# cbg-ethz/metMHN

Measured on AMD Instinct MI355X. Metric: full-cohort log-lik+grad evals/sec at n=20 events; kronvec HBM GB/s, higher is better.
Workload: dtype f64

## Files before the change

### include/metmhn_amd.h

```cpp
#ifndef METMHN_AMD_H
#define METMHN_AMD_H

#include <stddef.h>
#include <stdint.h>

#ifdef __cplusplus
extern "C" {
#endif

typedef struct mmhn_engine* mmhn_handle;

enum { MMHN_F64 = 0, MMHN_F32 = 1 };

int mmhn_create(int device_id, int n_mut, int dtype, mmhn_handle* out);
void mmhn_destroy(mmhn_handle h);
const char* mmhn_last_error(void);
int mmhn_set_workspace_limit(mmhn_handle h, size_t bytes);

int mmhn_set_cohort(mmhn_handle h, const int8_t* dat, int64_t n_pat, int n_cols);
int mmhn_score(mmhn_handle h, const double* log_theta, const double* log_d_p, const double* log_d_m,
               double perc_met, double* score);
int mmhn_score_and_grad(mmhn_handle h, const double* log_theta, const double* log_d_p,
                        const double* log_d_m, double perc_met, double* score, double* d_theta,
                        double* d_dp, double* d_dm);
// ... 59 lines not shown

enum { MMHN_ORD_OK = 0, MMHN_ORD_OVERFLOW = 1, MMHN_ORD_INVALID = 2, MMHN_ORD_TOO_LARGE = 3 };
enum { MMHN_ORD_BAD_STATUS = 1,
       MMHN_ORD_UNREACHABLE = 2,
       MMHN_ORD_NO_SEEDING = 3,
       MMHN_ORD_MT_PT_PART = 4,
       MMHN_ORD_MT_NO_SEEDING = 5,
       MMHN_ORD_ABSENT_MET = 6,
       MMHN_ORD_PRESENT_MET = 7 };
enum { MMHN_ORD_DEFAULT_FRONT_CAP = 64 };
int mmhn_likeliest_orders(mmhn_handle h, const double* log_theta, const double* obs1, const double* obs2,
                          const int8_t* dat, int64_t n_pat, int n_cols, int front_cap, int8_t* orders, double* prob,
                          int32_t* status);

enum { MMHN_K_OTHER_SOLVE = 0,
       MMHN_K_PSOLVE_FWD = 1,
       MMHN_K_PSOLVE_ADJ = 2,
       MMHN_K_PCLASS = 3,
       MMHN_K_CSOLVE_FWD = 4,
       MMHN_K_CSOLVE_ADJ = 5,
       MMHN_K_COUNT = 6 };
typedef struct {
  double ms;
  int64_t launches;
  double alg_bytes;
} mmhn_kernel_counter;
typedef struct {
  mmhn_kernel_counter kernel[MMHN_K_COUNT];
  double eval_ms;
  int64_t evals;
  int32_t comm_ranks;
  int32_t comm_rank;
} mmhn_counters;
#define MMHN_ABI_VERSION 7
int mmhn_abi_version(void);
int mmhn_bench_kronvec(mmhn_handle h, const double* log_theta, const int8_t* state, int64_t batch,
                       int iters, int transpose, int jacobi, double* ms_per_launch, int64_t* tiles);
int mmhn_bench_stream(mmhn_handle h, size_t bytes, int iters, int kind, double* gbps);
int mmhn_get_counters(mmhn_handle h, mmhn_counters* out);
int mmhn_reset_counters(mmhn_handle h);
int mmhn_debug_lane_moves(mmhn_handle h, int transposed, int* out);

#ifdef __cplusplus
}
#endif
#endif
```

### metmhn_amd/_lib.py

```python
from __future__ import annotations

import ctypes as C
import os
import subprocess

_HERE = os.path.dirname(os.path.abspath(__file__))
_ROOT = os.path.dirname(_HERE)
import glob
_SRC = [os.path.join(_HERE, "csrc", "engine.hip")] + sorted(glob.glob(os.path.join(_HERE, "csrc", "*.h")))
_HDR = os.path.join(_ROOT, "include", "metmhn_amd.h")
LIB_PATH = os.environ.get("MMHN_LIB", os.path.join(_HERE, "libmetmhn_amd.so"))

f64p = C.POINTER(C.c_double)
i8p = C.POINTER(C.c_int8)
i64p = C.POINTER(C.c_int64)
i32p = C.POINTER(C.c_int32)


KERNEL_CLASSES = ("other_solve", "psolve_fwd", "psolve_adj", "pclass", "csolve_fwd", "csolve_adj")


class KernelCounter(C.Structure):
    _fields_ = [("ms", C.c_double), ("launches", C.c_int64), ("alg_bytes", C.c_double)]

# ... 14 lines not shown
    "mmhn_cohort_sums_end": [C.c_void_p, f64p],
    "mmhn_cohort_wsums_begin": [C.c_void_p, f64p, f64p, f64p, C.c_int, C.c_double],
    "mmhn_cohort_wsums_end": [C.c_void_p, f64p],
    "mmhn_set_reduce_flag": [C.c_void_p, C.c_double],
    "mmhn_get_reduce_flag": [C.c_void_p, f64p],
    "mmhn_patient_grads": [C.c_void_p, f64p, f64p, f64p, f64p, f64p, f64p, f64p],
    "mmhn_kronvec": [C.c_void_p, f64p, i8p, f64p, f64p, C.c_int, C.c_int],
    "mmhn_kronvec_batched": [C.c_void_p, f64p, i8p, C.c_int64, f64p, f64p, C.c_int, C.c_int],
    "mmhn_jacobi_step_batched": [C.c_void_p, f64p, f64p, f64p, i8p, C.c_int64, f64p, f64p, f64p, C.c_int],
    "mmhn_kron_diag": [C.c_void_p, f64p, i8p, f64p],
    "mmhn_diag_scal": [C.c_void_p, f64p, i8p, f64p, f64p, C.c_int],
    "mmhn_obs_states": [C.c_void_p, i8p, C.c_int, i64p, i64p],
    "mmhn_resolvent": [C.c_void_p, f64p, f64p, f64p, i8p, f64p, f64p, C.c_int],
    "mmhn_x_partial_Q_y": [C.c_void_p, f64p, i8p, f64p, f64p, f64p],
    "mmhn_x_partial_D_y": [C.c_void_p, f64p, f64p, i8p, f64p, f64p, f64p, f64p],
    "mmhn_partial_diag_scal": [C.c_void_p, f64p, i8p, f64p, C.c_int, C.c_int, f64p],
    "mmhn_v_kronvec": [C.c_void_p, f64p, i8p, f64p, f64p, C.c_int, C.c_int],
    "mmhn_v_resolvent": [C.c_void_p, f64p, i8p, f64p, f64p, f64p, C.c_int],
    "mmhn_v_x_partial_Q_y": [C.c_void_p, f64p, i8p, f64p, f64p, f64p, f64p],
    "mmhn_v_kron_diag": [C.c_void_p, f64p, i8p, f64p, f64p],
    "mmhn_v_scal_d_pt": [C.c_void_p, f64p, f64p, i8p, f64p, f64p, f64p],
    "mmhn_v_d_scal_d_pt": [C.c_void_p, f64p, f64p, i8p, f64p, C.c_int, f64p, f64p],
    "mmhn_v_x_partial_D_y": [C.c_void_p, f64p, f64p, i8p, f64p, f64p, f64p, f64p],
    "mmhn_comm_unique_id": [C.c_void_p],
    "mmhn_comm_init": [C.c_void_p, C.c_void_p, C.c_int, C.c_int],
    "mmhn_comm_destroy": [C.c_void_p],
    "mmhn_bench_stream": [C.c_void_p, C.c_size_t, C.c_int, C.c_int, f64p],
    "mmhn_bench_kronvec": [C.c_void_p, f64p, i8p, C.c_int64, C.c_int, C.c_int, C.c_int, f64p, i64p],
    "mmhn_simulate": [C.c_void_p, f64p, f64p, f64p, C.c_int64, C.c_uint64, i8p, i8p],
    "mmhn_simulate_summary": [C.c_void_p, f64p, f64p, f64p, C.c_int64, C.c_int64, C.c_uint64, i64p],
    "mmhn_get_counters": [C.c_void_p, C.POINTER(Counters)],
    "mmhn_reset_counters": [C.c_void_p],
    "mmhn_debug_lane_moves": [C.c_void_p, C.c_int, C.POINTER(C.c_int)],
    "mmhn_likeliest_orders": [C.c_void_p, f64p, f64p, f64p, i8p, C.c_int64, C.c_int, C.c_int, i8p, f64p, i32p],
}
OTHER_SYMBOLS = ("mmhn_destroy", "mmhn_last_error", "mmhn_abi_version")
ABI_VERSION = 7


def needs_build() -> bool:
    if not os.path.exists(LIB_PATH):
        return True
    t = os.path.getmtime(LIB_PATH)
    return any(os.path.exists(s) and os.path.getmtime(s) > t for s in _SRC + [_HDR])


def build(force: bool = False, verbose: bool = False) -> str:
    if not force and not needs_build():
        return LIB_PATH
    hipcc = os.environ.get("HIPCC", "/opt/rocm/bin/hipcc")
    cmd = [hipcc, "-O3", "-std=c++17", "--offload-arch=gfx950", "-shared", "-fPIC", "-Wno-comment",
           "-o", LIB_PATH, _SRC[0]]
    if verbose:
        print(" ".join(cmd))
    res = subprocess.run(cmd, capture_output=True, text=True)
    if res.returncode != 0:
        raise RuntimeError("hipcc failed:\n" + res.stderr)
    return LIB_PATH


_lib = None


def load():
    global _lib
    if _lib is not None:
        return _lib
    if not os.path.exists(LIB_PATH):
        raise RuntimeError(
            f"{LIB_PATH} is missing: run `python -c 'import __graft_entry__ as g; g.build()'` "
# ... 30 lines not shown
```

### metmhn_amd/csrc/engine.hip

```cpp
#include <hip/hip_runtime.h>
#include <rccl/rccl.h>
#include <dlfcn.h>

#include <algorithm>
#include <chrono>
#include <cmath>
#include <cstdio>
#include <cstdlib>
#include <cstring>
#include <string>
#include <vector>

#include "../../include/metmhn_amd.h"
#include "kernels.h"
#include "tsolve.h"
#include "small.h"
#include "wsolve.h"
#include "wclass.h"
#include "sampler.h"

namespace mmhn {

static thread_local std::string g_err;

// ... 52 lines not shown

struct Staged {
  std::vector<int> pats, paired, probs;
  DevArr<int> d_pats, d_paired, d_probs;
  std::vector<int2> map, lmap;
  std::vector<int> lof;
  DevArr<int2> d_map, d_lmap;
  DevArr<int2> d_grc;
  CList cl[2];
  int maxk = 0;
  bool kind2 = false;
  bool empty() const { return pats.empty(); }
};

struct Batch {
  std::vector<PatRec> pats;
  std::vector<Desc> dJ, dS;
  std::vector<int2> mapJ, mapS;
  long long vecJ = 0, vecS = 0, asize = 0, tabJ = 0, tabS = 0;
  long long aclr = 0;
  int id = 0;
  int maxkJ = 0, maxkS = 0;
  int maxkcJ = 0;
  bool has_kind2 = false;
  std::vector<int2> lmapJ, lmapS;
  std::vector<int> lofJ, lofS;
  std::vector<int2> mapX;
  DevArr<int2> d_mapX;
  DevArr<int2> d_grc[4];
  DevArr<int2> d_grcJ;
  std::vector<int> sp_list[3][SP_NCLASS];
  DevArr<int> d_sp_list[3][SP_NCLASS];
  bool has_small = false;
  int mk1p = 9;
  Staged stg[2];
  std::vector<int> paired;
  DevArr<int> d_paired;
  std::vector<uint8_t> route;
  std::vector<int> olist;
  DevArr<int> d_olist;
  bool wpath = false;
  bool wdirect = false;
  std::vector<WDesc> wd;
  DevArr<WDesc> d_wd;
  int wnx = -1;
  std::vector<WChain> wchains;
  DevArr<WChain> d_wchains;
  long long offT = 0;
  CList clJ[2];
  std::vector<int2> lmapT;
  std::vector<int> lofT;
  DevArr<int2> d_lmapT;
  int maxkT = 0, maxkP = 0;
  int max_dl = 0;
  std::vector<int> ptoff;
  std::vector<uint32_t> ptiles;
  DevArr<int> d_ptoff;
  DevArr<uint32_t> d_ptiles;
  double seeded_bytes_P = 0;
  std::vector<int4> pcl;
  DevArr<int4> d_pcl;
  DevArr<PatRec> d_pats;
  DevArr<Desc> d_dJ, d_dS;
  DevArr<int2> d_mapJ, d_mapS, d_lmapJ, d_lmapS;
};

// ... 252 lines not shown
template <typename T>
struct Engine : EngineBase {
  int n = 0, N = 0;
  size_t ws_limit = 0;
  DevArr<Params<T>> d_par;
  Params<T>* h_par = nullptr;
  double* h_abi = nullptr;
  void* h_par_dev = nullptr;
  double* h_abi_dev = nullptr;
  bool zero_copy = true;
  bool time_kernels = true;
  std::vector<int8_t> dat;
  long long n_pat = 0;
  int n_cols = 0;
  std::vector<Batch> batches;
  double n_em = 0;
  DevArr<T> pi, lidgJ, qJ, rhsJ, rhsS, pS, lidgS, qS, seedS, GS, dots, bmJ, bmS, tabJ, tabS;
  DevArr<T> zarena;
  struct View { T* p = nullptr; } GJ, DJ, Abuf;
  static long long zarena_elems(long long nJ, long long asize, int N) { return up4(3 * nJ * N * N) + up4(3 * nJ * N) + up4(asize); }
  static long long zclear_elems(const Batch& b, int N) { return zarena_elems((long long)b.dJ.size(), b.aclr, N); }
  static long long up4(long long v) { return (v + 3) / 4 * 4; }
  int pi_owner = -1, qJ_owner = -1;
  DevArr<double> lp, out, sums, abi_sums, redbuf;
  DevArr<JLink<T>> links;
  ncclComm_t comm = nullptr;
  int comm_rank = 0, comm_size = 1;
  DevArr<uint16_t> d_perm;
  DevArr<int> d_lvl;
  bool use_jacobi = false;
  bool poison = false;
  hipStream_t side[3] = {};
  hipEvent_t ev_fork[3] = {}, ev_join[3] = {};
  bool small_path = true;
  int prep_split_max = 2048;
  int psolve_min = 384;
  int wsolve_min = 128;
  bool force_timing = false;
  bool coop_fault = false;
  int pcl_per = 16;
  int coop_wgs = 0;
  bool coop = true;
  DevArr<CoopCtl> coop_ctl;
  DevArr<unsigned> coop_flags[2];
  unsigned coop_epoch = 0;
  int coop_slot = 0;
  int cur_lane = 0;
  unsigned* h_abort = nullptr;
  unsigned* h_abort_dev = nullptr;
  int wsolve_wgs = 0;
  int wsolve_mode = 1;
  DevArr<T> piM, qM;
  int n_cu = 256;
  mmhn_counters cnt{};
  std::vector<std::pair<hipEvent_t, hipEvent_t>> ev_pool;
  size_t ev_used = 0;
  std::vector<double> ev_bytes;
  std::vector<int> ev_slot;

  Engine(int dev, int n_mut) : n(n_mut), N(n_mut + 1) {
    device = dev;
    cnt.comm_rank = -1;
    REQUIRE(n_mut >= 1 && n_mut < MAXN, "n_mut must be in [1, 31]");
    DevGuard guard(device);
    HIPCHECK(hipStreamCreateWithFlags(&stream, hipStreamNonBlocking));
    d_par.alloc(NPSET);
// ... 1 lines not shown
    HIPCHECK(hipHostGetDevicePointer(&h_par_dev, h_par, 0));
    static_assert(sizeof(Params<T>) % sizeof(uint4) == 0, "parameter block: whole 16-byte words");
    sums.alloc(2 * stride());
    size_t free_b = 0, total_b = 0;
    HIPCHECK(hipMemGetInfo(&free_b, &total_b));
    ws_limit = (size_t)(0.7 * (double)free_b);
    {
      std::vector<uint16_t> perm((size_t)(TB + 1) << TB, 0);
      std::vector<int> lvl((size_t)(TB + 1) * (TB + 2), 0);
      for (int t = 0; t <= TB; ++t) {
        int pos = 0;
        for (int l = 0; l <= t; ++l) {
          lvl[(size_t)t * (TB + 2) + l] = pos;
          for (uint32_t x = 0; x < (1u << t); ++x)
            if (popc(x) == l) perm[((size_t)t << TB) + pos++] = (uint16_t)x;
        }
        lvl[(size_t)t * (TB + 2) + t + 1] = pos;
      }
      d_perm.alloc(perm.size());
      d_lvl.alloc(lvl.size());
      HIPCHECK(hipMemcpy(d_perm.p, perm.data(), perm.size() * sizeof(uint16_t), hipMemcpyHostToDevice));
      HIPCHECK(hipMemcpy(d_lvl.p, lvl.data(), lvl.size() * sizeof(int), hipMemcpyHostToDevice));
      const char* sv = std::getenv("MMHN_SOLVER");
      use_jacobi = sv && std::string(sv) == "jacobi";
      if (const char* pm = std::getenv("MMHN_PSOLVE_MIN")) { psolve_min = std::atoi(pm); wsolve_min = psolve_min; }
      if (const char* pm = std::getenv("MMHN_WSOLVE_MIN")) wsolve_min = std::atoi(pm);
      if (const char* pm = std::getenv("MMHN_COOP")) coop = std::atoi(pm) != 0;
      if (const char* pm = std::getenv("MMHN_TIME_KERNELS")) force_timing = std::atoi(pm) != 0;
      if (const char* pm = std::getenv("MMHN_COOP_WGS")) coop_wgs = std::atoi(pm);
      if (const char* pm = std::getenv("MMHN_PCL_PER")) pcl_per = std::max(1, std::atoi(pm));
      if (const char* pm = std::getenv("MMHN_COOP_FAULT")) coop_fault = std::atoi(pm) != 0;
      if (const char* po = std::getenv("MMHN_POISON")) poison = std::atoi(po) != 0;
      if (const char* sp = std::getenv("MMHN_SMALL")) small_path = std::atoi(sp) != 0;
      if (const char* sp = std::getenv("MMHN_ZEROCOPY")) zero_copy = std::atoi(sp) != 0;
      if (const char* sp = std::getenv("MMHN_PREP_SPLIT")) prep_split_max = std::atoi(sp);
      if (const char* ms = std::getenv("MMHN_WSOLVE")) wsolve_mode = std::atoi(ms);
      if (const char* ms = std::getenv("MMHN_WSOLVE_WGS")) wsolve_wgs = std::atoi(ms);
      if (const char* sc = std::getenv("MMHN_SIM_CHUNK")) sim_chunk = std::max(1ll, std::atoll(sc));
      hipDeviceProp_t prop;
      HIPCHECK(hipGetDeviceProperties(&prop, device));
      n_cu = std::max(1, prop.multiProcessorCount);
    }
    HIPCHECK(hipFuncSetAttribute(reinterpret_cast<const void*>(&k_wsolve<T, false>), hipFuncAttributeMaxDynamicSharedMemorySize, (int)wsolve_lds<T>()));
    HIPCHECK(hipFuncSetAttribute(reinterpret_cast<const void*>(&k_wsolve<T, true>), hipFuncAttributeMaxDynamicSharedMemorySize, (int)wsolve_lds<T>()));
    HIPCHECK(hipFuncSetAttribute(reinterpret_cast<const void*>(&k_wsolve<T, false, WCfg<T>::NXT>), hipFuncAttributeMaxDynamicSharedMemorySize, (int)wsolve_lds<T>()));
    HIPCHECK(hipFuncSetAttribute(reinterpret_cast<const void*>(&k_wsolve<T, true, WCfg<T>::NXT>), hipFuncAttributeMaxDynamicSharedMemorySize, (int)wsolve_lds<T>()));
    HIPCHECK(hipFuncSetAttribute(reinterpret_cast<const void*>(&k_wclass<T>), hipFuncAttributeMaxDynamicSharedMemorySize, (int)wclass_lds<T>()));
    const int lds = 150 * 1024;
    HIPCHECK(hipFuncSetAttribute(reinterpret_cast<const void*>(&k_csolve<T, false, false>), hipFuncAttributeMaxDynamicSharedMemorySize, lds));
    HIPCHECK(hipFuncSetAttribute(reinterpret_cast<const void*>(&k_csolve<T, true, false>), hipFuncAttributeMaxDynamicSharedMemorySize, lds));
    HIPCHECK(hipFuncSetAttribute(reinterpret_cast<const void*>(&k_csolve<T, false, true>), hipFuncAttributeMaxDynamicSharedMemorySize, lds));
    HIPCHECK(hipFuncSetAttribute(reinterpret_cast<const void*>(&k_csolve<T, true, true>), hipFuncAttributeMaxDynamicSharedMemorySize, lds));
    HIPCHECK(hipFuncSetAttribute(reinterpret_cast<const void*>(&k_csolve<T, false, false, 4>), hipFuncAttributeMaxDynamicSharedMemorySize, lds));
    HIPCHECK(hipFuncSetAttribute(reinterpret_cast<const void*>(&k_csolve<T, true, false, 4>), hipFuncAttributeMaxDynamicSharedMemorySize, lds));
    coop_ctl.alloc(1);
    HIPCHECK(hipMemset(coop_ctl.p, 0, sizeof(CoopCtl)));
    HIPCHECK(hipHostMalloc(reinterpret_cast<void**>(&h_abort), 64, hipHostMallocDefault));
    HIPCHECK(hipHostGetDevicePointer(reinterpret_cast<void**>(&h_abort_dev), h_abort, 0));
    *h_abort = 0u;
    HIPCHECK(hipFuncSetAttribute(reinterpret_cast<const void*>(&k_spatient2<T>), hipFuncAttributeMaxDynamicSharedMemorySize, 160 * 1024));
    HIPCHECK(hipFuncSetAttribute(reinterpret_cast<const void*>(&k_spatient<T, 1024, 1>), hipFuncAttributeMaxDynamicSharedMemorySize, 160 * 1024));
    for (int i = 0; i < 3; ++i) {
      HIPCHECK(hipStreamCreateWithFlags(&side[i], hipStreamNonBlocking));
      HIPCHECK(hipEventCreateWithFlags(&ev_fork[i], hipEventDisableTiming));
      HIPCHECK(hipEventCreateWithFlags(&ev_join[i], hipEventDisableTiming));
    }
    HIPCHECK(hipFuncSetAttribute(reinterpret_cast<const void*>(&k_psolve2<T, false, true>), hipFuncAttributeMaxDynamicSharedMemorySize, lds));
    HIPCHECK(hipFuncSetAttribute(reinterpret_cast<const void*>(&k_psolve2<T, true, true>), hipFuncAttributeMaxDynamicSharedMemorySize, lds));
    HIPCHECK(hipFuncSetAttribute(reinterpret_cast<const void*>(&k_psolve2<T, false, false>), hipFuncAttributeMaxDynamicSharedMemorySize, lds));
    HIPCHECK(hipFuncSetAttribute(reinterpret_cast<const void*>(&k_psolve2<T, true, false>), hipFuncAttributeMaxDynamicSharedMemorySize, lds));
    HIPCHECK(hipFuncSetAttribute(reinterpret_cast<const void*>(&k_tsolve<T, false, false>), hipFuncAttributeMaxDynamicSharedMemorySize, lds));
    HIPCHECK(hipFuncSetAttribute(reinterpret_cast<const void*>(&k_tsolve<T, true, false>), hipFuncAttributeMaxDynamicSharedMemorySize, lds));
    HIPCHECK(hipFuncSetAttribute(reinterpret_cast<const void*>(&k_tsolve<T, false, true>), hipFuncAttributeMaxDynamicSharedMemorySize, lds));
    HIPCHECK(hipFuncSetAttribute(reinterpret_cast<const void*>(&k_tsolve<T, true, true>), hipFuncAttributeMaxDynamicSharedMemorySize, lds));
    HIPCHECK(hipFuncSetAttribute(reinterpret_cast<const void*>(&k_kv<T, false, 1, false>), hipFuncAttributeMaxDynamicSharedMemorySize, lds));
    HIPCHECK(hipFuncSetAttribute(reinterpret_cast<const void*>(&k_kv<T, true, 1, false>), hipFuncAttributeMaxDynamicSharedMemorySize, lds));
    HIPCHECK(hipFuncSetAttribute(reinterpret_cast<const void*>(&k_kv<T, false, 1, true>), hipFuncAttributeMaxDynamicSharedMemorySize, lds));
    HIPCHECK(hipFuncSetAttribute(reinterpret_cast<const void*>(&k_kv<T, true, 1, true>), hipFuncAttributeMaxDynamicSharedMemorySize, lds));
    HIPCHECK(hipFuncSetAttribute(reinterpret_cast<const void*>(&k_sweep<T, false>),
                                 hipFuncAttributeMaxDynamicSharedMemorySize, lds));
    HIPCHECK(hipFuncSetAttribute(reinterpret_cast<const void*>(&k_sweep<T, true>),
                                 hipFuncAttributeMaxDynamicSharedMemorySize, lds));
    HIPCHECK(hipFuncSetAttribute(reinterpret_cast<const void*>(&k_diag<T>),
                                 hipFuncAttributeMaxDynamicSharedMemorySize, lds));
    HIPCHECK(hipFuncSetAttribute(reinterpret_cast<const void*>(&k_diag<T, 1024>),
                                 hipFuncAttributeMaxDynamicSharedMemorySize, lds));
    HIPCHECK(hipFuncSetAttribute(reinterpret_cast<const void*>(&k_prep<T, false>), hipFuncAttributeMaxDynamicSharedMemorySize, lds));
    HIPCHECK(hipFuncSetAttribute(reinterpret_cast<const void*>(&k_prep<T, true>), hipFuncAttributeMaxDynamicSharedMemorySize, lds));
    HIPCHECK(hipFuncSetAttribute(reinterpret_cast<const void*>(&k_prep<T, false, 1024>), hipFuncAttributeMaxDynamicSharedMemorySize, lds));
    HIPCHECK(hipFuncSetAttribute(reinterpret_cast<const void*>(&k_grad_rows<T, 1>), hipFuncAttributeMaxDynamicSharedMemorySize, lds));
    HIPCHECK(hipFuncSetAttribute(reinterpret_cast<const void*>(&k_grad_rows<T>),
                                 hipFuncAttributeMaxDynamicSharedMemorySize, lds));
    HIPCHECK(hipFuncSetAttribute(reinterpret_cast<const void*>(&k_pclass<T, false>), hipFuncAttributeMaxDynamicSharedMemorySize, lds));
    HIPCHECK(hipFuncSetAttribute(reinterpret_cast<const void*>(&k_pclass<T, true>), hipFuncAttributeMaxDynamicSharedMemorySize, lds));
// ... 593 lines not shown
      bool class_fits[SP_NCLASS];
      for (int c = 0; c < SP_NCLASS; ++c)
        class_fits[c] = (spatient_lds<T>(N, spatient_class_maxk(c)) + 15) / 16 * 16 * (size_t)(c == 0 ? SP_PPB0 : c == 1 ? 2 : 1) + 64 <= (size_t)160 * 1024;
      const bool all_staged = !small_path || use_jacobi;
      for (size_t pi_ = 0; pi_ < b.pats.size(); ++pi_) {
        const PatRec& pr = b.pats[pi_];
        int ks = -1;
        for (int part = 0; part < 2; ++part) if (pr.s[part] >= 0) ks = std::max(ks, b.dS[pr.s[part]].k);
        if (ks < 0) continue;
        int c = 0;
        while (c < SP_NCLASS - 1 && ks > spatient_class_maxk(c)) ++c;
        if (all_staged || ks > TB || !class_fits[c]) {
          Staged& g = b.stg[all_staged || pr.j >= 0 ? 1 : 0];
          g.pats.push_back((int)pi_);
          if (pr.j >= 0) g.paired.push_back((int)pi_);
          for (int part = 0; part < 2; ++part) if (pr.s[part] >= 0) g.probs.push_back(pr.s[part]);
          if (pr.kind == 2) g.kind2 = true;
          continue;
        }
        const bool side_by_side = pr.j >= 0 && pr.s[0] >= 0 && pr.s[1] >= 0 && c < 2;
        b.sp_list[side_by_side ? 2 : pr.j >= 0 ? 1 : 0][c].push_back((int)pi_);
      }
      b.mk1p = spatient_class_maxk(1);
      if (!b.sp_list[1][2].empty() && b.sp_list[1][2].size() <= 16) {
        int mk = 0;
        for (int pi_ : b.sp_list[1][2])
          for (int part = 0; part < 2; ++part) if (b.pats[pi_].s[part] >= 0) mk = std::max(mk, b.dS[b.pats[pi_].s[part]].k);
        if (mk <= 10 && (spatient_lds<T>(N, mk) + 15) / 16 * 16 * 2 + 64 <= (size_t)160 * 1024) {
          for (int pi_ : b.sp_list[1][2]) b.sp_list[b.pats[pi_].s[0] >= 0 && b.pats[pi_].s[1] >= 0 ? 2 : 1][1].push_back(pi_);
          b.sp_list[1][2].clear();
          b.mk1p = mk;
        }
      }
      {
        auto ksize = [&](int pi_) {
          const PatRec& pr = b.pats[pi_];
          int ks = 0;
          for (int part = 0; part < 2; ++part) if (pr.s[part] >= 0) ks = std::max(ks, 64 * b.dS[pr.s[part]].k + (pr.s[0] >= 0 && pr.s[1] >= 0 ? 32 : 0) + pr.kind);
          return ks;
        };
        for (int w = 0; w < 3; ++w)
          for (int c = 0; c < SP_NCLASS; ++c)
            std::stable_sort(b.sp_list[w][c].begin(), b.sp_list[w][c].end(), [&](int x, int y) { return ksize(x) > ksize(y); });
      }
      b.has_small = false;
      for (int w = 0; w < 3; ++w)
        for (int c = 0; c < SP_NCLASS; ++c) {
          if (!b.sp_list[w][c].empty()) b.has_small = true;
          up(b.d_sp_list[w][c], b.sp_list[w][c]);
        }
      for (int w = 0; w < 2; ++w) {
        Staged& g = b.stg[w];
        std::vector<char> isg(b.dS.size(), 0);
        for (int sp : g.probs) isg[sp] = 1;
        g.map.clear(); g.maxk = 0;
        for (const int2& m : b.mapS) if (isg[m.x]) { g.map.push_back(m); g.maxk = std::max(g.maxk, b.dS[m.x].k); }
        build_levels(g.map, nullptr, false, g.lmap, g.lof);
        g.cl[0].clear(); g.cl[1].clear();
        if (!use_jacobi && g.lof.size() > 2) { build_clist(g.map, b.dS, false, false, g.cl[0]); build_clist(g.map, b.dS, false, true, g.cl[1]); }
        up(g.d_pats, g.pats); up(g.d_paired, g.paired); up(g.d_probs, g.probs);
        up(g.d_map, g.map); up(g.d_lmap, g.lmap);
        std::vector<int2> gc;
        for (const int2& e : grad_chunks(b.dS, GK_S)) if (isg[e.x]) gc.push_back(e);
        up(g.d_grc, gc);
      }
      b.wdirect = b.wpath && wsolve_mode != 2;
// ... 17 lines not shown
          up(b.d_grc[kd], gc);
          if (kd != GK_S) for (int2 e : gc) all.push_back(int2{e.x, e.y | (kd << 24)});
        }
        up(b.d_grcJ, all);
      }
      mvJ = std::max(mvJ, b.vecJ); mvS = std::max(mvS, b.vecS);
      mZ = std::max<size_t>(mZ, (size_t)zarena_elems((long long)b.dJ.size(), b.asize, N));
      mtJ = std::max(mtJ, b.tabJ); mtS = std::max(mtS, b.tabS);
      if (b.wpath && !b.wdirect) mvM = std::max(mvM, b.vecJ);
      mnJ = std::max(mnJ, b.dJ.size()); mnS = std::max(mnS, b.dS.size()); mp = std::max(mp, b.pats.size());
    }
    pi.alloc(mvJ); qJ.alloc(mvJ);
    piM.alloc(mvM); qM.alloc(mvM);
    if (use_jacobi) { lidgJ.alloc(mvJ); rhsJ.alloc(mvJ); }
    links.alloc(std::max<size_t>(mnJ, 1));
    tabJ.alloc(mtJ); tabS.alloc(mtS);
    pi_owner = qJ_owner = -1;
    rhsS.alloc(mvS); pS.alloc(mvS); lidgS.alloc(mvS); qS.alloc(mvS);
    seedS.alloc(mnS);
    GS.alloc(mnS * N * N); zarena.alloc(mZ);
    dots.alloc(2 * mp); bmJ.alloc(mnJ * 64); bmS.alloc(mnS * 64);
    lp.alloc(mp); out.alloc(mp * stride()); redbuf.alloc(((mp + red_per((int)mp) - 1) / red_per((int)mp)) * 2 * (size_t)stride());
  }

  bool small_forked[2] = {false, false}, fork_recorded[2] = {false, false};
  void small_fork(int which) {
    HIPCHECK(hipEventRecord(ev_fork[which], stream));
    fork_recorded[which] = true;
  }
  void small_classes(const Batch& b, int which, bool grad) {
    const int n0 = (int)b.sp_list[which][0].size(), n1 = (int)b.sp_list[which][1].size(), n2 = (int)b.sp_list[which][2].size();
    const int np0 = which ? (int)b.sp_list[2][0].size() : 0, np1 = which ? (int)b.sp_list[2][1].size() : 0;
    const int mk0 = spatient_class_maxk(0), mk1 = which ? b.mk1p : spatient_class_maxk(1), mk2 = spatient_class_maxk(2);
    const bool on_side = which == 0 ? (n0 + n1 + n2 > 0) : n2 > 0;
    hipStream_t sd = side[which];
    if (on_side) {
      if (!fork_recorded[which]) HIPCHECK(hipEventRecord(ev_fork[which], stream));
      HIPCHECK(hipStreamWaitEvent(sd, ev_fork[which], 0));
    }
    fork_recorded[which] = false;
#define SP_TAIL b.d_pats.p, b.d_dS.p, d_par.p, d_perm.p, d_lvl.p, b.d_dJ.p, b.d_wd.p, pi.p, links.p, pS.p, qS.p, GS.p, bmS.p, dots.p, lp.p
    auto big_class = [&]() {
      if (!n2) return;
      const size_t lds = (spatient_lds<T>(N, mk2) + 15) / 16 * 16;
      hipLaunchKernelGGL((k_spatient<T, 1024, 1>), dim3(n2), dim3(1024), lds, sd, b.d_sp_list[which][2].p, n2, SP_TAIL, mk2, N, grad ? 1 : 0);
      HIPCHECK(hipGetLastError());
    };
    big_class();
    if (n0 + n1 + np0 + np1) {
      const size_t s0 = (spatient_lds<T>(N, mk0) + 15) / 16 * 16, s1 = (spatient_lds<T>(N, mk1) + 15) / 16 * 16;
      const size_t lds = std::max(s0 * SP_PPB0, n1 + np1 ? s1 * (np1 ? 2 : 1) : 0) + 64;
      const int nblk = (n0 + SP_PPB0 - 1) / SP_PPB0 + n1 + (np0 + SP_PPB0 / 2 - 1) / (SP_PPB0 / 2) + np1;
      hipLaunchKernelGGL((k_spatient2<T>), dim3(nblk), dim3(256), lds, which == 0 ? sd : stream,
                         b.d_sp_list[which][0].p, n0, mk0, b.d_sp_list[which][1].p, n1, mk1,
                         b.d_sp_list[2][0].p, np0, b.d_sp_list[2][1].p, np1, SP_TAIL, N, grad ? 1 : 0);
      HIPCHECK(hipGetLastError());
    }
#undef SP_TAIL
    if (on_side) HIPCHECK(hipEventRecord(ev_join[which], sd));
    small_forked[which] = on_side;
  }
  void small_join(int which) {
    if (small_forked[which]) HIPCHECK(hipStreamWaitEvent(stream, ev_join[which], 0));
    small_forked[which] = false;
  }

  void evaluate(const double* lt, const double* ldp, const double* ldm, bool grad, double* host_sums,
                double* host_out) {
    REQUIRE(!sums_pending, "an evaluation begun with mmhn_cohort_sums_begin has not been collected");
    auto t0 = std::chrono::steady_clock::now();
    const int st = stride();
    small_forked[0] = small_forked[1] = fork_recorded[0] = fork_recorded[1] = false;
    bool head_done = false;
    if (zero_copy && !batches.empty()) {
      build_params(lt, ldp, ldm, false);
// ... 1243 lines not shown
  GUARD(h);
  unsigned long long v[16];
  HIPCHECK(hipDeviceSynchronize());
  HIPCHECK(hipMemcpyFromSymbol(v, HIP_SYMBOL(g_stamps), sizeof(v)));
  for (int i = 0; i < 16; ++i) out16[i] = (double)v[i];
  if (reset) { std::memset(v, 0, sizeof(v)); HIPCHECK(hipMemcpyToSymbol(HIP_SYMBOL(g_stamps), v, sizeof(v))); }
  API_END
}
#endif
int mmhn_get_counters(mmhn_handle h, mmhn_counters* out) {
  API_BEGIN
  GUARD(h);
  REQUIRE(h && h->impl && out, "null pointer");
  if (h->dtype == MMHN_F64) *out = static_cast<Engine<double>*>(h->impl)->cnt;
  else *out = static_cast<Engine<float>*>(h->impl)->cnt;
  API_END
}
int mmhn_debug_lane_moves(mmhn_handle h, int transposed, int* out) {
  API_BEGIN
  GUARD(h);
  REQUIRE(out, "null pointer");
  DevArr<int> d;
  d.alloc(6 * 64);
  if (transposed) hipLaunchKernelGGL((k_lane_moves<true>), dim3(1), dim3(64), 0, h->impl->stream, d.p);
  else hipLaunchKernelGGL((k_lane_moves<false>), dim3(1), dim3(64), 0, h->impl->stream, d.p);
  HIPCHECK(hipGetLastError());
  HIPCHECK(hipMemcpyAsync(out, d.p, 6 * 64 * sizeof(int), hipMemcpyDeviceToHost, h->impl->stream));
  HIPCHECK(hipStreamSynchronize(h->impl->stream));
  API_END
}

int mmhn_abi_version(void) { return MMHN_ABI_VERSION; }

int mmhn_reset_counters(mmhn_handle h) {
  API_BEGIN
  GUARD(h);
  DISPATCH(h, reset_counters());
  API_END
}

}
```

### metmhn_amd/csrc/small.h

```cpp
#pragma once
#include "kernels.h"

namespace mmhn {

constexpr int SP_NCLASS = 3;
constexpr int SP_PPB0 = 4;
__host__ __device__ inline int spatient_class_maxk(int c) { return c == 0 ? 6 : c == 1 ? 9 : TB; }
__host__ __device__ inline int spatient_lstride(int maxk) { return maxk < 6 ? 1 << maxk : 64; }
__host__ __device__ inline int spatient_rows(int maxk) { return maxk > 6 ? 1 << (maxk - 6) : 1; }

template <typename T>
__host__ __device__ inline size_t spatient_lds(int N, int maxk) {
  return ((size_t)N * (spatient_lstride(maxk) + spatient_rows(maxk) + 16 + 1) + 4 * 64 + 2 * 16 + ((size_t)3 << maxk) + 64) * sizeof(T) +
         (64 + TB + 2) * sizeof(int) + 8 + DESC_PAD + (sizeof(uint16_t) << maxk);
}

template <typename T, int SPB, int PPB, bool PAIR = false>
__device__ __forceinline__ void spatient_body(const int* __restrict__ plist, int npl, const PatRec* __restrict__ pats, const Desc* __restrict__ dS,
                                              const Params<T>* __restrict__ par,
                                              const uint16_t* __restrict__ perm, const int* __restrict__ lvl,
                                              const Desc* __restrict__ dJ, const WDesc* __restrict__ wds, const T* __restrict__ pi, JLink<T>* __restrict__ links,
                                              T* __restrict__ pS, T* __restrict__ qS,
                                              T* __restrict__ GS, T* __restrict__ bmS, T* __restrict__ dots,
                                              double* __restrict__ lp, int maxk, int N, int with_grad, int block) {
  constexpr int SPW = SPB / 64;
  static_assert(PAIR ? (PPB == 2 || (SPB == 64 && PPB % 2 == 0)) : (PPB == 1 || SPB == 64),
                "several patients per workgroup: one wave each; a pair of problems: two slots");
  extern __shared__ __align__(16) unsigned char smem_all[];
  const int pslot = PPB == 1 ? 0 : (int)(threadIdx.x / SPB);
  const size_t slot_bytes = (spatient_lds<T>(N, maxk) + 15) / 16 * 16;
  unsigned char* smem = smem_all + (size_t)pslot * slot_bytes;
  T* xch = reinterpret_cast<T*>(smem_all + (size_t)PPB * slot_bytes);
  const int mypart = pslot & 1;
  auto sync = [&]() {
    if (SPB == 64) { __builtin_amdgcn_fence(__ATOMIC_ACQ_REL, "wavefront"); __builtin_amdgcn_wave_barrier(); }
    else __syncthreads();
  };
  const int RS = spatient_rows(maxk);
  const int LS = spatient_lstride(maxk);
  T* Lc = reinterpret_cast<T*>(smem);
  T* Uc = Lc + N * LS;
  T* LA = Uc + N * RS;
  T* UA = LA + 64;
  T* LB = UA + 64;
  T* UB = LB + 64;
  T* P0 = UB + 64;
  T* Qv = P0 + ((size_t)1 << maxk);
  T* LID = Qv + ((size_t)1 << maxk);
  T* red = LID + ((size_t)1 << maxk);
  T* thl = red + 64;
  T* basel = thl + N * 16;
  T* dpl = basel + N;
  T* dml = dpl + 16;
  int* lev = reinterpret_cast<int*>(dml + 16);
  int* loff = lev + 64;
  Desc& dsh = *reinterpret_cast<Desc*>((reinterpret_cast<uintptr_t>(loff + TB + 2) + 7u) & ~(uintptr_t)7u);
  uint16_t* pml = reinterpret_cast<uint16_t*>(reinterpret_cast<unsigned char*>(&dsh) + DESC_PAD);
  const int pidx = PAIR ? block * (PPB / 2) + (pslot >> 1) : block * PPB + pslot;
  if (pidx >= npl) { if (PAIR && SPB == 64) __syncthreads(); return; }
  const int pat = plist[pidx];
  const PatRec pr = pats[pat];
  const int ps0 = pr.s[0], ps1 = pr.s[1];
  if (pr.kind == 4 || (PAIR ? (ps0 < 0 || ps1 < 0) : (ps0 < 0 && ps1 < 0))) { if (PAIR && SPB == 64) __syncthreads(); return; }
  const int kwalk = (PAIR && SPB > 64) ? max(dS[ps0].k, dS[ps1].k) : -1;
  const int tid = (int)(threadIdx.x % SPB), lane = tid & 63, w = tid >> 6;
  const int n = N - 1;

  auto setup = [&](const Desc& dg) {
    sync();
    {
      const int* sw = reinterpret_cast<const int*>(&dg);
      int* dw = reinterpret_cast<int*>(&dsh);
      for (int i = tid; i < DESC_WORDS; i += SPB) dw[i] = sw[i];
    }
    sync();
    const Desc& d = dsh;
    const int k = d.k;
    const Params<T>& P = par[d.pset];
    const int nl = k < 6 ? k : 6;
    const int R = k > 6 ? 1 << (k - 6) : 1;
    if (tid < k) { lev[tid] = d.ev[tid]; dpl[tid] = P.dp[d.ev[tid]]; dml[tid] = P.dm[d.ev[tid]]; }
    for (int e = tid; e < N * k; e += SPB) { const int i = e / k, b = e % k; thl[i * 16 + b] = P.th[i][d.ev[b]]; }
    for (int i = tid; i < N; i += SPB) basel[i] = P.baseP[i];
    if (SPB > 64) {
      const uint16_t* pm = perm + ((size_t)k << TB);
      for (uint32_t e = tid; e < (1u << k); e += SPB) pml[e] = pm[e];
      if (tid <= k + 1) loff[tid] = lvl[(size_t)k * (TB + 2) + tid];
    }
    sync();
    const int nL = 1 << nl;
    for (int e = tid; e < N * nL; e += SPB) {
      const int i = e >> nl, l = e & (nL - 1);
      T t[6];
#pragma unroll
      for (int bb = 0; bb < 6; ++bb) t[bb] = thl[i * 16 + bb];
      T v = 1;
#pragma unroll
// ... 94 lines not shown
    m.half = 1u << (k - 1);
    m.joff = dj->off;
    m.wl = dj->wl; m.kj = kj;
    m.free_is_row = m.wl >= 0 && (wds[m.wl].majP != 0) == (part == 1);
    return m;
  };
  auto marg_rhs = [&](const Marg& m, uint32_t x) -> T {
    if (x < m.half) return T(0);
    if (m.wl >= 0) return m.c * pi[m.joff + wpos_marg<T>(wds[m.wl], m.kj, m.free_is_row, x - m.half)];
    return m.c * pi[m.joff + (pdep32(x - m.half, m.free_) | m.fixed)];
  };
  Marg mg0{}, mg1{};

  STAMP_DECL;
  STAMP_START;
  T full_score = 0;
  for (int part = 0; part < 2; ++part) {
    const int sp = part == 0 ? ps0 : ps1;
    if (sp < 0 || (PAIR && part != mypart)) continue;
    setup(dS[sp]);
    STAMP(0);
    const Desc& d = dsh;
    const bool own = pr.kind <= 2;
    Marg mg{};
    if (!own) {
      mg = marg_of(part, d.k);
      if (part == 0) mg0 = mg; else mg1 = mg;
      if (tid == 0) { links[pr.j].soff[part] = d.off; links[pr.j].sk[part] = d.k; links[pr.j].cst[part] = mg.c; }
    }
    const bool stash = !PAIR && part == 1 && ps0 >= 0;
    T* yv = stash ? Qv : P0;
    solve(d, yv, false, [&](uint32_t x) { return own ? (x == 0 ? e0_scale<T>() : T(0)) : marg_rhs(mg, x); });
    full_score += yv[(1u << d.k) - 1u];
    if (stash) for (uint32_t x = tid; x < (1u << d.k); x += SPB) pS[d.off + x] = yv[x];
    STAMP(1);
  }
  if (pr.kind == 3 && !PAIR && tid == 0) {
    if (ps0 < 0) { links[pr.j].soff[0] = -1; links[pr.j].sk[0] = 0; links[pr.j].cst[0] = 0; }
    if (ps1 < 0) { links[pr.j].soff[1] = -1; links[pr.j].sk[1] = 0; links[pr.j].cst[1] = 0; }
  }
  if (PAIR) {
    if (tid == 0) xch[pslot] = full_score;
    __syncthreads();
    full_score = xch[pslot & ~1] + xch[pslot | 1];
  }
  const T seed = T(1) / full_score;
  if (tid == 0 && !(PAIR && mypart == 1)) {
    double l = log((double)full_score) - log((double)e0_scale<T>());
    if (pr.kind == 2) {
      const Desc& d = dsh;
      const Params<T>& P = par[PS_THETA];
      double dr = (double)P.dm[N - 1];
      for (int b = 0; b < d.k; ++b) if (b != d.seedbit) dr *= (double)dml[b];
      l += log(dr);
    }
    lp[pat] = l;
  }
  STAMP(2);
  if (!with_grad) { STAMP_FLUSH(0); return; }

  const int nparts = (ps0 >= 0) + (ps1 >= 0);
  for (int part = 0; part < 2; ++part) {
    const int sp = part == 0 ? ps0 : ps1;
    if (sp < 0 || (PAIR && part != mypart)) continue;
    if (nparts == 2 && !PAIR) setup(dS[sp]);
    const Desc& d = dsh;
    const int k = d.k;
    const uint32_t V = 1u << k, last = V - 1u;
    solve(d, Qv, true, [&](uint32_t x) { return x == last ? seed : T(0); });
    STAMP(3);
    if (!PAIR && part == 1 && ps0 >= 0) {
      sync();
      for (uint32_t x = tid; x < V; x += SPB) P0[x] = pS[d.off + x];
      sync();
    }
    const T* p = P0;
    if (pr.kind == 3) {
      T* qg = qS + d.off;
      const Marg& mg = part == 0 ? mg0 : mg1;
      const uint32_t half = V >> 1;
      T dot = 0;
      for (uint32_t x = tid; x < V; x += SPB) {
        const T qv = Qv[x];
        qg[x] = qv;
        if (x >= half) dot += qv * marg_rhs(mg, x);
      }
      dot = wave_sum_dpp(dot);
      if (lane == 0) red[w] = dot;
      sync();
      if (tid == 0) { T t = 0; for (int v = 0; v < SPW; ++v) t += red[v]; dots[2 * pat + part] = t; }
    }
    if (pr.kind == 2) {
      T* bm = bmS + (long long)sp * 64;
      const Params<T>& P0 = par[d.pset];
      T accA[TB], accB[TB];
#pragma unroll
      for (int b = 0; b < TB; ++b) { accA[b] = 0; accB[b] = 0; }
      for (uint32_t x = tid; x < V; x += SPB) {
        const uint32_t lo = x & 63u, ro = x >> 6;
        const bool sbit = d.seedbit >= 0 && ((x >> d.seedbit) & 1u);
        const T pq = p[x] * Qv[x];
        const T vA = sbit ? T(0) : pq * LA[lo] * UA[ro], vB = sbit ? pq * LB[lo] * UB[ro] * P0.dm[n] : T(0);
#pragma unroll
        for (int b = 0; b < TB; ++b) if (b < k && ((x >> b) & 1u)) { accA[b] += vA; accB[b] += vB; }
      }
      sync();
      T* part_ = LID;
// ... 74 lines not shown
            pv[u] = p[Sc]; q0[u] = Qv[Sc]; q1[u] = Qv[Sc | sb]; uc[u] = Uc[i * RS + (Sc >> 6)];
          }
#pragma unroll
          for (int u = 0; u < GU; ++u) {
            const uint32_t S0 = S00 + 64 * u, S = S0 + (uint32_t)lane;
            T a = -pv[u] * q0[u];
            if (slot >= 0) a += pv[u] * q1[u];
            const T f = (S < V && !(S & sb)) ? lcv * uc[u] * a : T(0);
            tot += f;
#pragma unroll
            for (int l = 0; l < TB - 6; ++l) if (l < nhi && ((S0 >> (6 + l)) & 1u)) hi[l] += f;
          }
        }
        T total, ML[6];
        wave_bit_sums(tot, lane, klo, total, ML);
        T mine = 0;
        if (lane == i) mine = total;
#pragma unroll
        for (int l = 0; l < 6; ++l)
          if (l < klo && lane == lev[l] && lev[l] != i) mine = ML[l];
#pragma unroll
        for (int h = 0; h < TB - 6; ++h) {
          if (h < nhi) {
            const T m = wave_sum_dpp(hi[h]);
            if (lane == lev[klo + h] && lev[klo + h] != i) mine = m;
          }
        }
        if (lane < N) G[i * N + lane] = mine;
      }
    }
    sync();
    STAMP(5);
  }
  STAMP_FLUSH(0);
}

#define SPATIENT_PARAMS const PatRec* __restrict__ pats, const Desc* __restrict__ dS, const Params<T>* __restrict__ par, \
    const uint16_t* __restrict__ perm, const int* __restrict__ lvl, const Desc* __restrict__ dJ, const WDesc* __restrict__ wds, \
    const T* __restrict__ pi, \
    JLink<T>* __restrict__ links, T* __restrict__ pS, \
    T* __restrict__ qS, T* __restrict__ GS, T* __restrict__ bmS, T* __restrict__ dots, double* __restrict__ lp
#define SPATIENT_ARGS pats, dS, par, perm, lvl, dJ, wds, pi, links, pS, qS, GS, bmS, dots, lp

template <typename T, int SPB, int PPB, bool PAIR = false>
__global__ __launch_bounds__(SPB * PPB) void k_spatient(const int* __restrict__ plist, int npl, SPATIENT_PARAMS, int maxk, int N,
                                                        int with_grad) {
  spatient_body<T, SPB, PPB, PAIR>(plist, npl, SPATIENT_ARGS, maxk, N, with_grad, (int)blockIdx.x);
}

template <typename T>
__global__ __launch_bounds__(256) void k_spatient2(const int* __restrict__ list0, int n0, int maxk0, const int* __restrict__ list1,
                                                   int n1, int maxk1, const int* __restrict__ pair0, int np0,
                                                   const int* __restrict__ pair1, int np1, SPATIENT_PARAMS, int N, int with_grad) {
  int b = (int)blockIdx.x;
  if (b < np1) { spatient_body<T, 128, 2, true>(pair1, np1, SPATIENT_ARGS, maxk1, N, with_grad, b); return; }
  b -= np1;
  if (b < n1) { spatient_body<T, 256, 1>(list1, n1, SPATIENT_ARGS, maxk1, N, with_grad, b); return; }
  b -= n1;
  const int nbp = (np0 + SP_PPB0 / 2 - 1) / (SP_PPB0 / 2);
  if (b < nbp) { spatient_body<T, 64, SP_PPB0, true>(pair0, np0, SPATIENT_ARGS, maxk0, N, with_grad, b); return; }
  spatient_body<T, 64, SP_PPB0>(list0, n0, SPATIENT_ARGS, maxk0, N, with_grad, b - nbp);
}
#undef SPATIENT_PARAMS
#undef SPATIENT_ARGS

}
```

Baseline: 22.23.

## Run both problems of big-class patients concurrently in one workgroup with per-slot LDS

Adds a k_spatient_big kernel that, for patients in the large class with two subproblems whose combined LDS fits in 160 KiB, runs both subproblems in parallel as two 512-thread halves of a 1024-thread workgroup. Each half gets an LDS slot sized to its own subproblem, and the Q/theta-local buffers are aliased to shrink the footprint. Unfitting patients keep the sequential 1024-thread path and are launched in the same grid. This trades fewer threads per subproblem for concurrency across the two parts, and adds a debug entry point that reports the LDS layout.

```diff
diff --git a/include/metmhn_amd.h b/include/metmhn_amd.h
--- a/include/metmhn_amd.h
+++ b/include/metmhn_amd.h
@@ -115,7 +115,7 @@
   int32_t comm_ranks;
   int32_t comm_rank;
 } mmhn_counters;
-#define MMHN_ABI_VERSION 7
+#define MMHN_ABI_VERSION 8
 int mmhn_abi_version(void);
 int mmhn_bench_kronvec(mmhn_handle h, const double* log_theta, const int8_t* state, int64_t batch,
                        int iters, int transpose, int jacobi, double* ms_per_launch, int64_t* tiles);
@@ -123,6 +123,7 @@
 int mmhn_get_counters(mmhn_handle h, mmhn_counters* out);
 int mmhn_reset_counters(mmhn_handle h);
 int mmhn_debug_lane_moves(mmhn_handle h, int transposed, int* out);
+int mmhn_debug_spatient_pair_lds(int n_events, int k0, int k1, int dtype, int64_t* out);
 
 #ifdef __cplusplus
 }
diff --git a/metmhn_amd/_lib.py b/metmhn_amd/_lib.py
--- a/metmhn_amd/_lib.py
+++ b/metmhn_amd/_lib.py
@@ -70,10 +70,11 @@
     "mmhn_get_counters": [C.c_void_p, C.POINTER(Counters)],
     "mmhn_reset_counters": [C.c_void_p],
     "mmhn_debug_lane_moves": [C.c_void_p, C.c_int, C.POINTER(C.c_int)],
+    "mmhn_debug_spatient_pair_lds": [C.c_int, C.c_int, C.c_int, C.c_int, i64p],
     "mmhn_likeliest_orders": [C.c_void_p, f64p, f64p, f64p, i8p, C.c_int64, C.c_int, C.c_int, i8p, f64p, i32p],
 }
 OTHER_SYMBOLS = ("mmhn_destroy", "mmhn_last_error", "mmhn_abi_version")
-ABI_VERSION = 7
+ABI_VERSION = 8
 
 
 def needs_build() -> bool:
diff --git a/metmhn_amd/csrc/engine.hip b/metmhn_amd/csrc/engine.hip
--- a/metmhn_amd/csrc/engine.hip
+++ b/metmhn_amd/csrc/engine.hip
@@ -108,6 +108,7 @@
   std::vector<int> sp_list[3][SP_NCLASS];
   DevArr<int> d_sp_list[3][SP_NCLASS];
   bool has_small = false;
+  size_t big_pair_lds = 0;
   int mk1p = 9;
   Staged stg[2];
   std::vector<int> paired;
@@ -426,6 +427,7 @@
   bool poison = false;
   hipStream_t side[3] = {};
   hipEvent_t ev_fork[3] = {}, ev_join[3] = {};
+  bool pair_big = true;
   bool small_path = true;
   int prep_split_max = 2048;
   int psolve_min = 384;
@@ -493,6 +495,7 @@
       if (const char* pm = std::getenv("MMHN_COOP_FAULT")) coop_fault = std::atoi(pm) != 0;
       if (const char* po = std::getenv("MMHN_POISON")) poison = std::atoi(po) != 0;
       if (const char* sp = std::getenv("MMHN_SMALL")) small_path = std::atoi(sp) != 0;
+      if (const char* sp = std::getenv("MMHN_SP_PAIR1024")) pair_big = std::atoi(sp) != 0;
       if (const char* sp = std::getenv("MMHN_ZEROCOPY")) zero_copy = std::atoi(sp) != 0;
       if (const char* sp = std::getenv("MMHN_PREP_SPLIT")) prep_split_max = std::atoi(sp);
       if (const char* ms = std::getenv("MMHN_WSOLVE")) wsolve_mode = std::atoi(ms);
@@ -521,6 +524,7 @@
     *h_abort = 0u;
     HIPCHECK(hipFuncSetAttribute(reinterpret_cast<const void*>(&k_spatient2<T>), hipFuncAttributeMaxDynamicSharedMemorySize, 160 * 1024));
     HIPCHECK(hipFuncSetAttribute(reinterpret_cast<const void*>(&k_spatient<T, 1024, 1>), hipFuncAttributeMaxDynamicSharedMemorySize, 160 * 1024));
+    HIPCHECK(hipFuncSetAttribute(reinterpret_cast<const void*>(&k_spatient_big<T>), hipFuncAttributeMaxDynamicSharedMemorySize, 160 * 1024));
     for (int i = 0; i < 3; ++i) {
       HIPCHECK(hipStreamCreateWithFlags(&side[i], hipStreamNonBlocking));
       HIPCHECK(hipEventCreateWithFlags(&ev_fork[i], hipEventDisableTiming));
@@ -1180,6 +1184,17 @@
           b.mk1p = mk;
         }
       }
+      b.big_pair_lds = 0;
+      if (pair_big) {
+        std::vector<int> seq;
+        for (int pi_ : b.sp_list[1][2]) {
+          const PatRec& pr = b.pats[pi_];
+          const size_t need = pr.s[0] >= 0 && pr.s[1] >= 0 ? spatient_pair_lds<T>(N, b.dS[pr.s[0]].k, b.dS[pr.s[1]].k) : SP_LDS_MAX + 1;
+          if (need <= SP_LDS_MAX) { b.sp_list[2][2].push_back(pi_); b.big_pair_lds = std::max(b.big_pair_lds, need); }
+          else seq.push_back(pi_);
+        }
+        b.sp_list[1][2].swap(seq);
+      }
       {
         auto ksize = [&](int pi_) {
           const PatRec& pr = b.pats[pi_];
@@ -1263,7 +1278,8 @@
     const int n0 = (int)b.sp_list[which][0].size(), n1 = (int)b.sp_list[which][1].size(), n2 = (int)b.sp_list[which][2].size();
     const int np0 = which ? (int)b.sp_list[2][0].size() : 0, np1 = which ? (int)b.sp_list[2][1].size() : 0;
     const int mk0 = spatient_class_maxk(0), mk1 = which ? b.mk1p : spatient_class_maxk(1), mk2 = spatient_class_maxk(2);
-    const bool on_side = which == 0 ? (n0 + n1 + n2 > 0) : n2 > 0;
+    const int np2 = which ? (int)b.sp_list[2][2].size() : 0;
+    const bool on_side = which == 0 ? (n0 + n1 + n2 > 0) : n2 + np2 > 0;
     hipStream_t sd = side[which];
     if (on_side) {
       if (!fork_recorded[which]) HIPCHECK(hipEventRecord(ev_fork[which], stream));
@@ -1272,6 +1288,13 @@
     fork_recorded[which] = false;
 #define SP_TAIL b.d_pats.p, b.d_dS.p, d_par.p, d_perm.p, d_lvl.p, b.d_dJ.p, b.d_wd.p, pi.p, links.p, pS.p, qS.p, GS.p, bmS.p, dots.p, lp.p
     auto big_class = [&]() {
+      if (np2) {
+        const size_t lds = std::max(b.big_pair_lds, n2 ? (spatient_lds<T>(N, mk2) + 15) / 16 * 16 : 0);
+        hipLaunchKernelGGL((k_spatient_big<T>), dim3(np2 + n2), dim3(1024), lds, sd, b.d_sp_list[2][2].p, np2, b.d_sp_list[1][2].p, n2,
+                           SP_TAIL, mk2, N, grad ? 1 : 0);
+        HIPCHECK(hipGetLastError());
+        return;
+      }
       if (!n2) return;
       const size_t lds = (spatient_lds<T>(N, mk2) + 15) / 16 * 16;
       hipLaunchKernelGGL((k_spatient<T, 1024, 1>), dim3(n2), dim3(1024), lds, sd, b.d_sp_list[which][2].p, n2, SP_TAIL, mk2, N, grad ? 1 : 0);
@@ -2581,6 +2604,27 @@
 
 int mmhn_abi_version(void) { return MMHN_ABI_VERSION; }
 
+int mmhn_debug_spatient_pair_lds(int n_events, int k0, int k1, int dtype, int64_t* out) {
+  API_BEGIN
+  REQUIRE(out, "null pointer");
+  REQUIRE(n_events >= 1 && n_events <= MAXN && k0 >= 0 && k0 <= TB && k1 >= 0 && k1 <= TB, "events in 1..32, bits in 0..12");
+  REQUIRE(dtype == MMHN_F64 || dtype == MMHN_F32, "dtype");
+  auto fill = [&](auto t) {
+    using T = decltype(t);
+    const size_t need = spatient_pair_lds<T>(n_events, k0, k1), s1 = spatient_pair_slot<T>(n_events, k0);
+    out[0] = (int64_t)need;
+    out[1] = need <= SP_LDS_MAX;
+    out[2] = (int64_t)s1;
+    out[3] = (int64_t)spatient_carve<T>(n_events, k0, true).end;
+    out[4] = (int64_t)(s1 + spatient_carve<T>(n_events, k1, true).end);
+    out[5] = (int64_t)(s1 + spatient_pair_slot<T>(n_events, k1) + 2 * sizeof(T));
+    out[6] = (int64_t)((spatient_lds<T>(n_events, TB) + 15) / 16 * 16);
+    out[7] = (int64_t)spatient_carve<T>(n_events, TB, false).end;
+  };
+  if (dtype == MMHN_F64) fill(double()); else fill(float());
+  API_END
+}
+
 int mmhn_reset_counters(mmhn_handle h) {
   API_BEGIN
   GUARD(h);
diff --git a/metmhn_amd/csrc/small.h b/metmhn_amd/csrc/small.h
--- a/metmhn_amd/csrc/small.h
+++ b/metmhn_amd/csrc/small.h
@@ -14,8 +14,44 @@
   return ((size_t)N * (spatient_lstride(maxk) + spatient_rows(maxk) + 16 + 1) + 4 * 64 + 2 * 16 + ((size_t)3 << maxk) + 64) * sizeof(T) +
          (64 + TB + 2) * sizeof(int) + 8 + DESC_PAD + (sizeof(uint16_t) << maxk);
 }
-
-template <typename T, int SPB, int PPB, bool PAIR = false>
+__host__ __device__ inline size_t spatient_qcap(int N, int k) { return ((size_t)1 << k) > (size_t)N * 16 ? (size_t)1 << k : (size_t)N * 16; }
+template <typename T>
+__host__ __device__ inline size_t spatient_lds_own(int N, int k) {
+  return ((size_t)N * (spatient_lstride(k) + spatient_rows(k) + 1) + 4 * 64 + 2 * 16 + ((size_t)2 << k) + spatient_qcap(N, k) + 64) * sizeof(T) +
+         (64 + TB + 2) * sizeof(int) + 8 + DESC_PAD + (sizeof(uint16_t) << k);
+}
+template <typename T>
+__host__ __device__ inline size_t spatient_pair_slot(int N, int k) { return (spatient_lds_own<T>(N, k) + 15) / 16 * 16; }
+template <typename T>
+__host__ __device__ inline size_t spatient_pair_lds(int N, int k0, int k1) { return spatient_pair_slot<T>(N, k0) + spatient_pair_slot<T>(N, k1) + 64; }
+constexpr size_t SP_LDS_MAX = (size_t)160 * 1024;
+
+struct SpCarve { uint32_t Lc, Uc, LA, UA, LB, UB, P0, Qv, LID, red, thl, basel, dpl, dml, lev, loff, dsh, pml, end; };
+template <typename T>
+__host__ __device__ inline SpCarve spatient_carve(int N, int maxk, bool own) {
+  SpCarve c;
+  const uint32_t E = sizeof(T), V = 1u << maxk;
+  c.Lc = 0;
+  c.Uc = c.Lc + E * N * spatient_lstride(maxk);
+  c.LA = c.Uc + E * N * spatient_rows(maxk);
+  c.UA = c.LA + E * 64; c.LB = c.UA + E * 64; c.UB = c.LB + E * 64;
+  c.P0 = c.UB + E * 64;
+  c.Qv = c.P0 + E * V;
+  c.LID = c.Qv + E * (own ? (uint32_t)spatient_qcap(N, maxk) : V);
+  c.red = c.LID + E * V;
+  c.thl = own ? c.Qv : c.red + E * 64;
+  c.basel = own ? c.red + E * 64 : c.thl + E * N * 16;
+  c.dpl = c.basel + E * N;
+  c.dml = c.dpl + E * 16;
+  c.lev = c.dml + E * 16;
+  c.loff = c.lev + 4 * 64;
+  c.dsh = (c.loff + 4 * (TB + 2) + 7u) & ~7u;
+  c.pml = c.dsh + DESC_PAD;
+  c.end = c.pml + (uint32_t)(sizeof(uint16_t) << maxk);
+  return c;
+}
+
+template <typename T, int SPB, int PPB, bool PAIR = false, bool OWN = false>
 __device__ __forceinline__ void spatient_body(const int* __restrict__ plist, int npl, const PatRec* __restrict__ pats, const Desc* __restrict__ dS,
                                               const Params<T>* __restrict__ par,
                                               const uint16_t* __restrict__ perm, const int* __restrict__ lvl,
@@ -26,36 +62,10 @@
   constexpr int SPW = SPB / 64;
   static_assert(PAIR ? (PPB == 2 || (SPB == 64 && PPB % 2 == 0)) : (PPB == 1 || SPB == 64),
                 "several patients per workgroup: one wave each; a pair of problems: two slots");
+  static_assert(!OWN || (PAIR && PPB == 2 && SPB > 64), "slots of their own size: one pair of problems to a workgroup");
   extern __shared__ __align__(16) unsigned char smem_all[];
   const int pslot = PPB == 1 ? 0 : (int)(threadIdx.x / SPB);
-  const size_t slot_bytes = (spatient_lds<T>(N, maxk) + 15) / 16 * 16;
-  unsigned char* smem = smem_all + (size_t)pslot * slot_bytes;
-  T* xch = reinterpret_cast<T*>(smem_all + (size_t)PPB * slot_bytes);
   const int mypart = pslot & 1;
-  auto sync = [&]() {
-    if (SPB == 64) { __builtin_amdgcn_fence(__ATOMIC_ACQ_REL, "wavefront"); __builtin_amdgcn_wave_barrier(); }
-    else __syncthreads();
-  };
-  const int RS = spatient_rows(maxk);
-  const int LS = spatient_lstride(maxk);
-  T* Lc = reinterpret_cast<T*>(smem);
-  T* Uc = Lc + N * LS;
-  T* LA = Uc + N * RS;
-  T* UA = LA + 64;
-  T* LB = UA + 64;
-  T* UB = LB + 64;
-  T* P0 = UB + 64;
-  T* Qv = P0 + ((size_t)1 << maxk);
-  T* LID = Qv + ((size_t)1 << maxk);
-  T* red = LID + ((size_t)1 << maxk);
-  T* thl = red + 64;
-  T* basel = thl + N * 16;
-  T* dpl = basel + N;
-  T* dml = dpl + 16;
-  int* lev = reinterpret_cast<int*>(dml + 16);
-  int* loff = lev + 64;
-  Desc& dsh = *reinterpret_cast<Desc*>((reinterpret_cast<uintptr_t>(loff + TB + 2) + 7u) & ~(uintptr_t)7u);
-  uint16_t* pml = reinterpret_cast<uint16_t*>(reinterpret_cast<unsigned char*>(&dsh) + DESC_PAD);
   const int pidx = PAIR ? block * (PPB / 2) + (pslot >> 1) : block * PPB + pslot;
   if (pidx >= npl) { if (PAIR && SPB == 64) __syncthreads(); return; }
   const int pat = plist[pidx];
@@ -63,6 +73,44 @@
   const int ps0 = pr.s[0], ps1 = pr.s[1];
   if (pr.kind == 4 || (PAIR ? (ps0 < 0 || ps1 < 0) : (ps0 < 0 && ps1 < 0))) { if (PAIR && SPB == 64) __syncthreads(); return; }
   const int kwalk = (PAIR && SPB > 64) ? max(dS[ps0].k, dS[ps1].k) : -1;
+  size_t slot_off, xch_off;
+  if (OWN) {
+    const int k0 = dS[ps0].k, k1 = dS[ps1].k;
+    maxk = mypart ? k1 : k0;
+    slot_off = mypart ? spatient_pair_slot<T>(N, k0) : 0;
+    xch_off = spatient_pair_slot<T>(N, k0) + spatient_pair_slot<T>(N, k1);
+  } else {
+    const size_t slot_bytes = (spatient_lds<T>(N, maxk) + 15) / 16 * 16;
+    slot_off = (size_t)pslot * slot_bytes;
+    xch_off = (size_t)PPB * slot_bytes;
+  }
+  unsigned char* smem = smem_all + slot_off;
+  T* xch = reinterpret_cast<T*>(smem_all + xch_off);
+  auto sync = [&]() {
+    if (SPB == 64) { __builtin_amdgcn_fence(__ATOMIC_ACQ_REL, "wavefront"); __builtin_amdgcn_wave_barrier(); }
+    else __syncthreads();
+  };
+  const int RS = spatient_rows(maxk);
+  const int LS = spatient_lstride(maxk);
+  const SpCarve cv = spatient_carve<T>(N, maxk, OWN);
+  T* Lc = reinterpret_cast<T*>(smem + cv.Lc);
+  T* Uc = reinterpret_cast<T*>(smem + cv.Uc);
+  T* LA = reinterpret_cast<T*>(smem + cv.LA);
+  T* UA = reinterpret_cast<T*>(smem + cv.UA);
+  T* LB = reinterpret_cast<T*>(smem + cv.LB);
+  T* UB = reinterpret_cast<T*>(smem + cv.UB);
+  T* P0 = reinterpret_cast<T*>(smem + cv.P0);
+  T* Qv = reinterpret_cast<T*>(smem + cv.Qv);
+  T* LID = reinterpret_cast<T*>(smem + cv.LID);
+  T* red = reinterpret_cast<T*>(smem + cv.red);
+  T* thl = reinterpret_cast<T*>(smem + cv.thl);
+  T* basel = reinterpret_cast<T*>(smem + cv.basel);
+  T* dpl = reinterpret_cast<T*>(smem + cv.dpl);
+  T* dml = reinterpret_cast<T*>(smem + cv.dml);
+  int* lev = reinterpret_cast<int*>(smem + cv.lev);
+  int* loff = reinterpret_cast<int*>(smem + cv.loff);
+  Desc& dsh = *reinterpret_cast<Desc*>(smem + cv.dsh);
+  uint16_t* pml = reinterpret_cast<uint16_t*>(smem + cv.pml);
   const int tid = (int)(threadIdx.x % SPB), lane = tid & 63, w = tid >> 6;
   const int n = N - 1;
 
@@ -223,8 +271,8 @@
     T* yv = stash ? Qv : P0;
     solve(d, yv, false, [&](uint32_t x) { return own ? (x == 0 ? e0_scale<T>() : T(0)) : marg_rhs(mg, x); });
     full_score += yv[(1u << d.k) - 1u];
-    if (stash) for (uint32_t x = tid; x < (1u << d.k); x += SPB) pS[d.off + x] = yv[x];
     STAMP(1);
+    if (stash) { for (uint32_t x = tid; x < (1u << d.k); x += SPB) pS[d.off + x] = yv[x]; STAMP(7); }
   }
   if (pr.kind == 3 && !PAIR && tid == 0) {
     if (ps0 < 0) { links[pr.j].soff[0] = -1; links[pr.j].sk[0] = 0; links[pr.j].cst[0] = 0; }
@@ -248,13 +296,13 @@
     lp[pat] = l;
   }
   STAMP(2);
-  if (!with_grad) { STAMP_FLUSH(0); return; }
+  if (!with_grad) { STAMP_FLUSH(PAIR ? 8 : 0); return; }
 
   const int nparts = (ps0 >= 0) + (ps1 >= 0);
   for (int part = 0; part < 2; ++part) {
     const int sp = part == 0 ? ps0 : ps1;
     if (sp < 0 || (PAIR && part != mypart)) continue;
-    if (nparts == 2 && !PAIR) setup(dS[sp]);
+    if (nparts == 2 && !PAIR) { setup(dS[sp]); STAMP(6); }
     const Desc& d = dsh;
     const int k = d.k;
     const uint32_t V = 1u << k, last = V - 1u;
@@ -264,6 +312,7 @@
       sync();
       for (uint32_t x = tid; x < V; x += SPB) P0[x] = pS[d.off + x];
       sync();
+      STAMP(7);
     }
     const T* p = P0;
     if (pr.kind == 3) {
@@ -404,7 +453,7 @@
     sync();
     STAMP(5);
   }
-  STAMP_FLUSH(0);
+  STAMP_FLUSH(PAIR ? 8 : 0);
 }
 
 #define SPATIENT_PARAMS const PatRec* __restrict__ pats, const Desc* __restrict__ dS, const Params<T>* __restrict__ par, \
@@ -418,6 +467,14 @@
 __global__ __launch_bounds__(SPB * PPB) void k_spatient(const int* __restrict__ plist, int npl, SPATIENT_PARAMS, int maxk, int N,
                                                         int with_grad) {
   spatient_body<T, SPB, PPB, PAIR>(plist, npl, SPATIENT_ARGS, maxk, N, with_grad, (int)blockIdx.x);
+}
+
+template <typename T>
+__global__ __launch_bounds__(1024) void k_spatient_big(const int* __restrict__ pairs, int np, const int* __restrict__ list, int nl,
+                                                       SPATIENT_PARAMS, int maxk, int N, int with_grad) {
+  const int b = (int)blockIdx.x;
+  if (b < np) { spatient_body<T, 512, 2, true, true>(pairs, np, SPATIENT_ARGS, 0, N, with_grad, b); return; }
+  spatient_body<T, 1024, 1>(list, nl, SPATIENT_ARGS, maxk, N, with_grad, b - np);
 }
 
 template <typename T>
```

New measurement: 22.24 (median of 4 runs). Within noise of the previous version (+0.0%).
